# CNR-STIIMA-IRAS/rosdyn

Hardware: NVIDIA B200
Metric: 6-DOF regressor+torque samples/sec (fp64) (higher is better)
Workload: dtype f64

## Files before the change

### rosdyn_b200/csrc/gram_common.cuh

```cuda
#pragma once
#ifndef __CUDACC_RTC__
#include <cuda_runtime.h>
#endif

#include "chain_dev.h"
#include "spatial.cuh"

namespace rdb
{

constexpr int GF_KSPLIT = 4;
constexpr int GF_MMA_WARPS = 2 * GF_KSPLIT;
constexpr int GF_GENS = GF_KSPLIT;
constexpr int GF_THREADS = 32 * (GF_MMA_WARPS + GF_GENS);
constexpr int GF_MAX_SLOTS = 4;
constexpr int GF_BAR_REDUCE = 1;

__device__ __forceinline__ void bar_sync(int id, int count) { asm volatile("bar.sync %0, %1;" ::"r"(id), "r"(count) : "memory"); }
__device__ __forceinline__ void dmma884f(double& d0, double& d1, double a, double b)
{
  asm volatile("mma.sync.aligned.m8n8k4.row.col.f64.f64.f64.f64 {%0,%1}, {%2}, {%3}, {%0,%1};\n" : "+d"(d0), "+d"(d1) : "d"(a), "d"(b));
}
__device__ __forceinline__ uint32_t smem_u32(const void* p) { return (uint32_t)__cvta_generic_to_shared(p); }

template <int V>
struct ic
{
  static constexpr int value = V;
};
template <int B, int E, class F>
__device__ __forceinline__ void static_for(F&& f)
{
  if constexpr (B < E)
  {
    f(ic<B>{});
    static_for<B + 1, E>(f);
  }
}

constexpr int GX_COLS = 8;
template <int NJ, int Z = 0>
struct GramGeom
{
  static constexpr int P = 10 * NJ;
  static constexpr int TC = Z == 2 ? 0 : 1;
  __host__ __device__ static constexpr int inblk(int p)
  {
    constexpr int zord[10] = {9, 1, 2, 8, 3, 4, 5, 6, 7, 0};
    return Z == 2 ? zord[p] : (Z == 1 ? (p == 0 ? 9 : p - 1) : p);
  }
  __host__ __device__ static constexpr int param_at(int q)
  {
    constexpr int zinv[10] = {9, 1, 2, 4, 5, 6, 7, 8, 3, 0};
    return Z == 2 ? zinv[q] : (Z == 1 ? (q == 9 ? 0 : q + 1) : q);
  }
  __host__ __device__ static constexpr int pos(int l, int p) { return TC + 10 * (NJ - 1 - l) + inblk(p); }
  __host__ __device__ static constexpr bool stored(int j, int l, int p)
  {
    if (j != l || Z == 0) return true;
    if (Z == 1) return p != 0;
    return l == 0 ? (p == 1 || p == 2 || p == 9) : (p != 0 && p != 3);
  }
  __host__ __device__ static constexpr int rowlen(int j)
  {
    return Z == 2 ? TC + 10 * (NJ - 1 - j) + (j == 0 ? 3 : 8) : 1 + 10 * (NJ - j) - Z;
  }
  static constexpr int NPOS = rowlen(0);
  __host__ __device__ static constexpr int col_of(int q) { return q < TC ? P : 10 * (NJ - 1 - (q - TC) / 10) + param_at((q - TC) % 10); }
  __host__ __device__ static constexpr bool has_pos(int c) { return c / 10 > 0 || stored(0, 0, c % 10); }
  static constexpr int T = (NPOS + 7) / 8;
  static constexpr int NT = T * (T + 1) / 2;
  static constexpr int NF = T + 1 - TC;
  static constexpr int PARTIAL = NT * 64 + (TC ? 0 : 8 * T + 1);
  static constexpr int KPW = 8 / GF_KSPLIT;
  static constexpr int NSTEPS = NJ * KPW;
  __host__ __device__ static constexpr int rowbase(int j)
  {
    int o = 0;
    for (int i = 0; i < j; i++) o += rowlen(i) * 32;
    return o;
  }
  __host__ __device__ static constexpr int taubase(int j) { return TC ? rowbase(j) : rowbase(NJ) + 32 * j; }
  static constexpr int SLOT_DOUBLES = rowbase(NJ) + (TC ? 0 : 32 * NJ);
  __host__ __device__ static constexpr int tile(int I, int J) { return I * T - I * (I - 1) / 2 + (J - I); }
  __host__ __device__ static constexpr bool owns(int I, int par) { return (I & 1) == par; }
  __host__ __device__ static constexpr int ntiles(int par)
  {
    int n = 0;
    for (int I = 0; I < T; I++)
      if (owns(I, par)) n += T - I;
    return n > 0 ? n : 1;
  }
  __host__ __device__ static constexpr int local(int I, int J, int par)
  {
    int n = 0;
    for (int K = 0; K < I; K++)
      if (owns(K, par)) n += T - K;
    return n + (J - I);
  }
  __host__ __device__ static constexpr int bown(int I, int par)
  {
    int n = 0;
    for (int K = 0; K < I; K++)
      if (owns(K, par)) n++;
    return n;
  }
  __host__ __device__ static constexpr int nbacc(int par) { return TC || (par != 0 && bown(T, par) == 0) ? 1 : bown(T, par) + (par == 0 ? 1 : 0); }
  __host__ __device__ static constexpr int tj(int j) { return (rowlen(j) + 7) / 8; }
  __host__ __device__ static constexpr int xtile(int j, int I)
  {
    int n = 0;
    for (int k = 0; k < j; k++) n += tj(k) + 1;
    return n + I;
  }
  __host__ __device__ static constexpr int nxt()
  {
    int n = 0;
    for (int k = 0; k < NJ; k++) n += tj(k) + 1;
    return n;
  }
  static constexpr int NXT = nxt();
  __host__ __device__ static constexpr bool xowns(int j, int I, int par) { return ((I == tj(j) ? j : I) & 1) == par; }
  __host__ __device__ static constexpr int xlocal(int j, int I, int par)
  {
    int n = 0;
    for (int k = 0; k <= j; k++)
      for (int K = 0; K <= tj(k); K++)
      {
        if (k == j && K == I) return n;
        if (xowns(k, K, par)) n++;
      }
    return n;
  }
  __host__ __device__ static constexpr int nxtiles(int par)
  {
    int n = 0;
    for (int k = 0; k < NJ; k++)
      for (int K = 0; K <= tj(k); K++)
        if (xowns(k, K, par)) n++;
    return n;
  }
};

enum : int
{
  GXK_SAT = 1,
  GXK_OMEGA = 2,
  GXK_SGN = 3,
  GXK_SQ = 4,
  GXK_Q = 5,
  GXK_ONE = 6
};
struct GramComps
{
  int32_t ncols[8];
  int32_t kind[8][GX_COLS];
  double thr[8][GX_COLS], vmax[8][GX_COLS];
  double ithr[8][GX_COLS];
};

struct RtModel
{
  static constexpr bool RUNTIME = true;
};
enum : int
{
  MK_A = 0,
  MK_T = 1,
  MK_PI = 2,
  MK_G = 3
};
struct Zr
{
};
template <int S>
struct Un
{
};
template <class T>
struct tv_unit
{
  static constexpr int s = 0;
};
template <int S>
struct tv_unit<Un<S>>
{
  static constexpr int s = S;
};
template <class T>
struct tv_zero
{
  static constexpr bool v = false;
};
template <>
struct tv_zero<Zr>
{
  static constexpr bool v = true;
};

template <class M, int F, int L, int K, int NJ>
__device__ __forceinline__ auto kc(const ChainDev<NJ>& C)
{
  if constexpr (M::RUNTIME)
  {
    if constexpr (F == MK_A) return C.joint[L].A[K];
    else if constexpr (F == MK_T) return C.joint[L].t[K];
    else if constexpr (F == MK_PI) return C.link[L].pi[K];
    else return C.g[K];
  }
  else
  {
    constexpr double v = M::val(F, L, K);
    if constexpr (v == 0.0) return Zr{};
    else if constexpr (v == 1.0) return Un<1>{};
    else if constexpr (v == -1.0) return Un<-1>{};
    else return v;
  }
}

template <class A>
__device__ __forceinline__ double tv_d(A a)
{
  if constexpr (tv_zero<A>::v) return 0.0;
  else if constexpr (tv_unit<A>::s != 0) return (double)tv_unit<A>::s;
  else return a;
}
template <class A>
__device__ __forceinline__ auto tneg(A a)
{
  if constexpr (tv_zero<A>::v) return Zr{};
  else if constexpr (tv_unit<A>::s != 0) return Un<-tv_unit<A>::s>{};
  else return -a;
}
template <class A, class B>
__device__ __forceinline__ auto tmul(A a, B b)
{
  constexpr int ua = tv_unit<A>::s, ub = tv_unit<B>::s;
  if constexpr (tv_zero<A>::v || tv_zero<B>::v) return Zr{};
  else if constexpr (ua != 0 && ub != 0) return Un<ua * ub>{};
  else if constexpr (ua != 0) return ua > 0 ? b : -b;
  else if constexpr (ub != 0) return ub > 0 ? a : -a;
  else return __dmul_rn(a, b);
}
template <class A, class B>
__device__ __forceinline__ auto tadd(A a, B b)
{
  if constexpr (tv_zero<A>::v) return b;
  else if constexpr (tv_zero<B>::v) return a;
  else return __dadd_rn(tv_d(a), tv_d(b));
}
template <class A, class B, class C>
__device__ __forceinline__ auto tfma(A a, B b, C c)
{
  using P = decltype(tmul(a, b));
  if constexpr (tv_zero<P>::v) return c;
  else if constexpr (tv_zero<C>::v) return tmul(a, b);
  else if constexpr (tv_unit<A>::s != 0 || tv_unit<B>::s != 0) return tadd(tmul(a, b), c);
  else return __fma_rn(a, b, tv_d(c));
}

// ... 75 lines not shown
    if (G::stored(J, L, p))
      o[G::pos(L, p) * 32 + (lane ^ (4 * (G::pos(L, p) & 3)))] = e[p];
}
template <class M, int NJ, int Z, int L, int J, class U, class S>
__device__ __forceinline__ void gram_project(const ChainDev<NJ>& C, double (&tau)[NJ], double* __restrict__ slot, int lane, const U& u, const S& s,
                                             const V3& fm, const V3& w, const V3& al)
{
  const auto h = tcross_add(tcross_add(tcross(u, al), w, tcross(w, u)), fm, s);
  const auto rho = tcross(s, w);
  gram_emit<M, NJ, Z, L, J, false>(
      C, tau, slot, lane, tdot(u, fm), h.x, h.y, h.z, tfma(s.x, al.x, tmul(rho.x, w.x)),
      tfma(s.x, al.y, tfma(s.y, al.x, tfma(rho.x, w.y, tmul(rho.y, w.x)))), tfma(s.x, al.z, tfma(s.z, al.x, tfma(rho.x, w.z, tmul(rho.z, w.x)))),
      tfma(s.y, al.y, tmul(rho.y, w.y)), tfma(s.y, al.z, tfma(s.z, al.y, tfma(rho.y, w.z, tmul(rho.z, w.y)))), tfma(s.z, al.z, tmul(rho.z, w.z)));
}

template <int NJ, class M, int Z>
__device__ __forceinline__ void gram_walk_rev(const ChainDev<NJ>& C, const GenIn<NJ>& x, double* __restrict__ slot, int lane, double (&tau)[NJ])
{
  static_assert(REV_AXIS[0] == 0.0 && REV_AXIS[1] == 0.0 && REV_AXIS[2] == 1.0, "the REV walk below is written for the axis s = e_z");
  V3 U[NJ], S[NJ];
  V3 v = v3(0, 0, 0), w = v3(0, 0, 0), a = v3(0, 0, 0), al = v3(0, 0, 0), g;
  static_for<0, NJ>([&](auto lc) {
    constexpr int l = decltype(lc)::value;
    const double dql = x.dq[l], ddql = x.ddq[l];
    const double sl = x.sv[l], cl = x.cv[l];
    const auto t = mk3(kc<M, MK_T, l, 0>(C), kc<M, MK_T, l, 1>(C), kc<M, MK_T, l, 2>(C));
    auto row = [&](auto kc_) {
      constexpr int k = decltype(kc_)::value;
      const auto a0 = kc<M, MK_A, l, 3 * k>(C);
      const auto a1 = kc<M, MK_A, l, 3 * k + 1>(C);
      return mk3(tfma(sl, a1, tmul(cl, a0)), tfma(-sl, a0, tmul(cl, a1)), kc<M, MK_A, l, 3 * k + 2>(C));
    };
    const auto R = mk3(row(ic<0>{}), row(ic<1>{}), row(ic<2>{}));
    v = tod3(trotT(R, tcross_add(v, w, t)));
    w = tod3(trotT(R, w));
    a = tod3(trotT(R, tcross_add(a, al, t)));
    al = tod3(trotT(R, al));
    if constexpr (l == 0) g = tod3(trotT(R, mk3(kc<M, MK_G, 0, 0>(C), kc<M, MK_G, 0, 1>(C), kc<M, MK_G, 0, 2>(C))));
    else g = tod3(trotT(R, g));
    w.z += dql;
    a.x = fma(v.y, dql, a.x);
    a.y = fma(-v.x, dql, a.y);
    al.x = fma(w.y, dql, al.x);
    al.y = fma(-w.x, dql, al.y);
    al.z += ddql;
    static_for<0, (l > 0 ? l - 1 : 0)>([&](auto jc) {
      constexpr int j = decltype(jc)::value;
      U[j] = tod3(trotT(R, tcross_add(U[j], S[j], t)));
      S[j] = tod3(trotT(R, S[j]));
    });
    const auto S1 = R.z;
    const auto U1 = mk3(tfma(t.x, R.y.x, tneg(tmul(t.y, R.x.x))), tfma(t.x, R.y.y, tneg(tmul(t.y, R.x.y))), tfma(t.x, R.y.z, tneg(tmul(t.y, R.x.z))));
    if constexpr (l > 0)
    {
      S[l - 1] = tod3(S1);
      U[l - 1] = tod3(U1);
    }
    const V3 fm = cross_add(a - g, w, v);
    static_for<0, l + 1>([&](auto jc) {
      constexpr int j = decltype(jc)::value;
      if constexpr (j == l)
      {
        const double e7 = w.x * w.y;
        gram_emit<M, NJ, Z, l, j, true>(C, tau, slot, lane, Zr{}, fm.y, -fm.x, Zr{}, -e7, fma(w.x, w.x, -(w.y * w.y)), fma(-w.y, w.z, al.x),
                                        e7, fma(w.x, w.z, al.y), al.z);
      }
      else if constexpr (j == l - 1) gram_project<M, NJ, Z, l, j>(C, tau, slot, lane, U1, S1, fm, w, al);
      else gram_project<M, NJ, Z, l, j>(C, tau, slot, lane, U[j], S[j], fm, w, al);
    });
  });
}

template <int NJ, int Z>
__device__ __forceinline__ void gram_walk_gen(const ChainDev<NJ>& C, const GenIn<NJ>& x, double* __restrict__ slot, int lane, double (&tau)[NJ])
{
  using G = GramGeom<NJ, Z>;
  V3 U[NJ], S[NJ];
  V3 v = v3(0, 0, 0), w = v3(0, 0, 0), a = v3(0, 0, 0), al = v3(0, 0, 0);
  V3 g = v3(C.g);
#pragma unroll
  for (int l = 0; l < NJ; l++)
  {
    const JointDev& J = C.joint[l];
    const double dql = x.dq[l], ddql = x.ddq[l];
    double R[9];
    const V3 t = J.type != RDB_JOINT_PRISMATIC ? v3(J.t) : axpy(v3(J.t), v3(J.axp), x.q[l]);
    if (J.type == RDB_JOINT_REVOLUTE)
    {
      const double c1 = 1.0 - x.cv[l];
#pragma unroll
      for (int k = 0; k < 9; k++) R[k] = fma(c1, J.C[k], fma(x.sv[l], J.B[k], J.A[k]));
    }
    else
    {
#pragma unroll
      for (int k = 0; k < 9; k++) R[k] = J.A[k];
    }
    v = rotT(R, cross_add(v, w, t));
    w = rotT(R, w);
    a = rotT(R, cross_add(a, al, t));
    al = rotT(R, al);
    g = rotT(R, g);
    const V3 axj = v3(J.ax);
    const V3 su = J.type == RDB_JOINT_PRISMATIC ? axj : v3(0, 0, 0);
    const V3 ss = J.type == RDB_JOINT_REVOLUTE ? axj : v3(0, 0, 0);
    v = axpy(v, su, dql);
    w = axpy(w, ss, dql);
    const V3 xl = cross_add(cross(w, su), v, ss);
    const V3 xa = cross(w, ss);
    a = axpy(axpy(a, xl, dql), su, ddql);
    al = axpy(axpy(al, xa, dql), ss, ddql);
    U[l] = su;
    S[l] = ss;
#pragma unroll
    for (int j = 0; j < l; j++)
    {
      U[j] = rotT(R, cross_add(U[j], S[j], t));
      S[j] = rotT(R, S[j]);
    }
    tau[l] = 0.0;
    const double* Pl = C.link[l].pi;
    const V3 fm = cross_add(a - g, w, v);
#pragma unroll
    for (int j = 0; j <= l; j++)
    {
      const V3 u = U[j], s = S[j];
      const V3 h = cross_add(cross_add(cross(u, al), w, cross(w, u)), fm, s);
      const V3 rho = cross(s, w);
      double e[10];
      e[0] = dot(u, fm);
      e[1] = h.x;
      e[2] = h.y;
      e[3] = h.z;
      e[4] = fma(s.x, al.x, rho.x * w.x);
      e[5] = fma(s.x, al.y, fma(s.y, al.x, fma(rho.x, w.y, rho.y * w.x)));
      e[6] = fma(s.x, al.z, fma(s.z, al.x, fma(rho.x, w.z, rho.z * w.x)));
      e[7] = fma(s.y, al.y, rho.y * w.y);
      e[8] = fma(s.y, al.z, fma(s.z, al.y, fma(rho.y, w.z, rho.z * w.y)));
      e[9] = fma(s.z, al.z, rho.z * w.z);
      double t0 = tau[j], t1 = e[1] * Pl[1];
#pragma unroll
      for (int p = 0; p < 10; p += 2) t0 = fma(e[p], Pl[p], t0);
#pragma unroll
      for (int p = 3; p < 10; p += 2) t1 = fma(e[p], Pl[p], t1);
      tau[j] = t0 + t1;
      double* o = slot + G::rowbase(j);
#pragma unroll
      for (int p = 0; p < 10; p++) o[G::pos(l, p) * 32 + (lane ^ (4 * (G::pos(l, p) & 3)))] = e[p];
    }
  }
}

template <int NJ, bool REV, int Z, class M>
__device__ __forceinline__ void gram_generate(const ChainDev<NJ>& C, const GenIn<NJ>& x, const SamplesDev& in, const double* __restrict__ tau_meas,
                                              double* __restrict__ slot, int64_t i, int lane)
{
  static_assert(!Z || REV, "the zero mass column of a link on its own joint exists for revolute joints only");
  static_assert(REV || M::RUNTIME, "compile-time models are built for the REV walk");
  using G = GramGeom<NJ, Z>;
  double tau[NJ];
  if constexpr (REV) gram_walk_rev<NJ, M, Z>(C, x, slot, lane, tau);
  else gram_walk_gen<NJ, Z>(C, x, slot, lane, tau);
#pragma unroll
  for (int j = 0; j < NJ; j++)
  {
    const double tv = tau_meas ? __ldcs(tau_meas + (int64_t)C.joint[j].in * in.ld + i) : tau[j];
    slot[G::taubase(j) + lane] = tv;
  }
}

template <int NJ, int Z>
__device__ __noinline__ void gram_zero_lane(double* __restrict__ slot, int lane)
{
  using G = GramGeom<NJ, Z>;
  for (int j = 0; j < NJ; j++)
  {
    for (int c = 0; c < G::rowlen(j); c++) slot[G::rowbase(j) + c * 32 + (lane ^ (4 * (c & 3)))] = 0.0;
    if (!G::TC) slot[G::taubase(j) + lane] = 0.0;
  }
}

}
```

### rosdyn_b200/csrc/gram_fused.cu

```cuda
#include <cuda_runtime.h>

#include <algorithm>
#include <cstdio>
#include <cstdlib>
#include <type_traits>
#include <vector>

#include "gram_fused.cuh"
#include "launch.h"

namespace rdb
{

template <int NJ, int Z>
__global__ void gram_fused_reduce_kernel(const double* __restrict__ partial, int nparts, int pstride, double* __restrict__ gram,
                                         double* __restrict__ rhs, double* __restrict__ tau_sq, int accumulate)
{
  using G = GramGeom<NJ, Z>;
  constexpr int P = G::P;
  const int e = blockIdx.x * blockDim.x + threadIdx.x;
  if (!accumulate && e < P * (P + 1))
  {
    const int c = e / (P + 1), r = e % (P + 1);
    if (!G::has_pos(c))
    {
      if (r == P) rhs[c] = 0.0;
      else
      {
        gram[(size_t)c * P + r] = 0.0;
        gram[(size_t)r * P + c] = 0.0;
      }
    }
  }
  if (e >= G::PARTIAL) return;
  double s = 0.0;
  for (int p = 0; p < nparts; p++) s += partial[(size_t)p * pstride + e];
  if (e >= G::NT * 64)
  {
    const int q = e - G::NT * 64;
    if (q == 8 * G::T)
    {
      if (tau_sq) *tau_sq = accumulate ? *tau_sq + s : s;
    }
    else if (q < G::NPOS)
    {
      const int a = G::col_of(q);
      rhs[a] = accumulate ? rhs[a] + s : s;
    }
    return;
  }
  int k = e >> 6, I = 0;
  while (k >= G::T - I)
  {
    k -= G::T - I;
    I++;
  }
  const int J = I + k;
  const int rp = 8 * I + ((e >> 3) & 7), cp = 8 * J + (e & 7);
  if (rp >= G::NPOS || cp >= G::NPOS) return;
  if (I == J && rp > cp) return;
  const int row = G::col_of(rp), col = G::col_of(cp);
  if (row < P && col < P)
  {
    const double v = accumulate ? gram[(size_t)col * P + row] + s : s;
    gram[(size_t)col * P + row] = v;
    if (row != col) gram[(size_t)row * P + col] = v;
  }
  else if (row < P || col < P)
  {
    const int a = row < P ? row : col;
    rhs[a] = accumulate ? rhs[a] + s : s;
  }
  else if (tau_sq)
    *tau_sq = accumulate ? *tau_sq + s : s;
}
template <int NJ, int Z>
static void launch_fused_reduce(const double* partial, int nparts, int pstride, double* gram, double* rhs, double* tau_sq, int accumulate,
                                cudaStream_t st)
{
  using G = GramGeom<NJ, Z>;
  const int n = std::max(G::PARTIAL, G::P * (G::P + 1));
  gram_fused_reduce_kernel<NJ, Z><<<(n + 255) / 256, 256, 0, st>>>(partial, nparts, pstride, gram, rhs, tau_sq, accumulate);
  count_launch();
}

__global__ void gram_fold_expand_kernel(const double* __restrict__ T, const int32_t* __restrict__ kof, const double* __restrict__ Gr,
                                        const double* __restrict__ br, const double* __restrict__ tsr, int nj, int Pr, double* __restrict__ gram,
                                        double* __restrict__ rhs, double* __restrict__ tau_sq, int accumulate)
{
  const int P = 10 * nj;
  const int e = blockIdx.x * blockDim.x + threadIdx.x;
  if (e >= P * (P + 1)) return;
  const int a = e / (P + 1), b = e % (P + 1);
  if (e == P && tau_sq) *tau_sq = accumulate ? *tau_sq + *tsr : *tsr;
  if (b < a) return;
  const int la = a / 10, pa = a % 10, ka = kof[la];
  double s = 0.0;
  if (b == P)
  {
    if (ka >= 0)
      for (int c = 0; c < 10; c++) s = fma(T[(size_t)la * 100 + c * 10 + pa], br[10 * ka + c], s);
    rhs[a] = accumulate ? rhs[a] + s : s;
    return;
  }
  const int lb = b / 10, pb = b % 10, kb = kof[lb];
  if (ka >= 0 && kb >= 0)
    for (int c = 0; c < 10; c++)
    {
      double r = 0.0;
      for (int d = 0; d < 10; d++) r = fma(Gr[(size_t)(10 * kb + d) * Pr + 10 * ka + c], T[(size_t)lb * 100 + d * 10 + pb], r);
      s = fma(T[(size_t)la * 100 + c * 10 + pa], r, s);
    }
  const double v = accumulate ? gram[(size_t)b * P + a] + s : s;
  gram[(size_t)b * P + a] = v;
  if (a != b) gram[(size_t)a * P + b] = v;
}

static int gram_dev_switch()
{
#ifdef RDB_DEV_SWITCHES
  static const int dbg = [] { const char* e = getenv("RDB_GRAM_DEBUG"); return e ? atoi(e) : 0; }();
  return dbg;
#else
  return 0;
#endif
}

cudaError_t launch_fold_expand(ChainHost& ch, double* gram, double* rhs, double* tau_sq, int accumulate, cudaStream_t st)
{
  const int nj = ch.host.nj, Pr = 10 * ch.gram.fold.nj, P = 10 * nj;
  double* Tm = ch.gram.fold_dev;
  double* Gr = Tm + (size_t)nj * 100;
  double* br = Gr + (size_t)Pr * Pr;
  double* tsr = br + Pr;
  const int32_t* kof = reinterpret_cast<const int32_t*>(Gr + (size_t)(Pr + 1) * (Pr + 1));
  gram_fold_expand_kernel<<<(P * (P + 1) + 127) / 128, 128, 0, st>>>(Tm, kof, Gr, br, tsr, nj, Pr, gram, rhs, tau_sq, accumulate);
  count_launch();
  return cudaGetLastError();
}

template <int NJ>
static ChainDev<NJ> narrow_g(const ChainDev<RDB_MAX_JOINTS>& h)
{
  ChainDev<NJ> c;
  c.nj = h.nj;
  c.n_in = h.n_in;
  for (int k = 0; k < 3; k++) c.g[k] = h.g[k];
  for (int j = 0; j < NJ; j++)
  {
    c.joint[j] = h.joint[j];
    c.link[j] = h.link[j];
  }
  return c;
}

static cudaError_t grow(double*& p, size_t& have, size_t need)
{
  if (have >= need) return cudaSuccess;
  if (p) cudaFree(p);
  p = nullptr;
  have = 0;
  cudaError_t e = cudaMalloc(&p, need);
  if (e == cudaSuccess) have = need;
  return e;
}

template <int NJ, int Z, int XC>
constexpr int gf_slots()
{
  return std::min<int>(GF_MAX_SLOTS,
                       (int)((227 * 1024 - 1024) / (sizeof(double) * (GramGeom<NJ, Z>::SLOT_DOUBLES + gram_ext_side_doubles<NJ, XC>()))));
}

template <int NJ, bool REV, int XC>
static cudaError_t launch_fused_kernel(ChainHost& ch, const GramComps& gc, const SamplesDev& in, const double* tau_meas, double* partials,
                                       int* grid, cudaStream_t st)
{
  constexpr int Z = REV ? (XC ? 1 : 2) : 0;
  constexpr int SLOTS = gf_slots<NJ, Z, XC>();
  static_assert(SLOTS >= 2, "the fused kernel needs two slots");
  const void* kfn = reinterpret_cast<const void*>(gram_fused_kernel<NJ, SLOTS, REV, XC>);
  if (REV)
  {
    char args[64];
    snprintf(args, sizeof args, "gram_fused_kernel<%d, %d, true, %d", NJ, SLOTS, XC);
    if (const void* jk = gram_jit_kernel(ch, args)) kfn = jk;
  }
  else
  {
    ch.gram.kernel_specialised = 0;
    ch.gram.kernel_why = "precompiled kernel: not every folded joint is revolute about e_z (generic generator)";
  }
  const size_t smem = sizeof(double) * (size_t)gram_smem_doubles<NJ, Z, SLOTS, XC>();
  cudaError_t e = cudaFuncSetAttribute(kfn, cudaFuncAttributeMaxDynamicSharedMemorySize, (int)smem);
  if (e != cudaSuccess) return e;
  const int64_t ngroups = (in.n + 31) / 32;
  constexpr int B = gram_group_block<SLOTS, XC>();
  *grid = (int)std::min<int64_t>(ch.sm_count, (ngroups + B - 1) / B);
  ChainDev<NJ> C = narrow_g<NJ>(ch.gram.fold);
  GramComps comps = gc;
  SamplesDev ins = in;
  const double* tm = tau_meas;
  double* part = partials;
  int dbg = gram_dev_switch();
  void* args[] = {&C, &comps, &ins, &tm, &part, &dbg};
  e = cudaLaunchKernel(kfn, dim3(*grid), dim3(GF_THREADS), args, smem, st);
  if (e != cudaSuccess) return e;
  count_launch();
  return cudaSuccess;
}

template <int NJ, bool REV>
static cudaError_t launch_fused_nj(ChainHost& ch, const SamplesDev& in, const double* tau_meas, double* gram, double* rhs, double* tau_sq,
                                   int accumulate, cudaStream_t st)
{
  constexpr int Z = REV ? 2 : 0;
  using G = GramGeom<NJ, Z>;
  cudaError_t e = grow(ch.gram.fused_partials, ch.gram.fused_bytes, sizeof(double) * (size_t)ch.sm_count * G::PARTIAL);
  if (e != cudaSuccess) return e;
  int grid = 0;
  e = launch_fused_kernel<NJ, REV, 0>(ch, GramComps{}, in, tau_meas, ch.gram.fused_partials, &grid, st);
  if (e != cudaSuccess) return e;
  if (ch.gram.fold_identity)
  {
    launch_fused_reduce<NJ, Z>(ch.gram.fused_partials, grid, G::PARTIAL, gram, rhs, tau_sq, accumulate, st);
    return cudaGetLastError();
  }
  const int nj = ch.host.nj, Pr = G::P;
  double* Tm = ch.gram.fold_dev;
  double* Gr = Tm + (size_t)nj * 100;
  double* br = Gr + (size_t)Pr * Pr;
  double* tsr = br + Pr;
  launch_fused_reduce<NJ, Z>(ch.gram.fused_partials, grid, G::PARTIAL, Gr, br, tsr, 0, st);
  return launch_fold_expand(ch, gram, rhs, tau_sq, accumulate, st);
}

cudaError_t launch_gram_fused(ChainHost& ch, const SamplesDev& in, const double* tau_meas, double* gram, double* rhs, double* tau_sq,
                              int accumulate, cudaStream_t st)
{
  if (in.n <= 0 || ch.gram.fold_version != ch.model_version) return cudaErrorNotSupported;
  const bool rev = fold_rev_canonical(ch.gram.fold);
  switch (ch.gram.fold.nj)
  {
#define X(N)                                                                                  \
  case N:                                                                                     \
    return rev ? launch_fused_nj<N, true>(ch, in, tau_meas, gram, rhs, tau_sq, accumulate, st) \
               : launch_fused_nj<N, false>(ch, in, tau_meas, gram, rhs, tau_sq, accumulate, st);
    X(1) X(2) X(3) X(4) X(5) X(6) X(7)
#undef X
  }
  return cudaErrorNotSupported;
}

__global__ void gram_cross_reduce_kernel(const double* __restrict__ partial, int nparts, int n, int pstride, double* __restrict__ sum)
{
  const int e = blockIdx.x * blockDim.x + threadIdx.x;
  if (e >= n) return;
  double s = 0.0;
  for (int p = 0; p < nparts; p++) s += partial[(size_t)p * pstride + e];
  sum[e] = s;
}

__global__ void gram_ext_scatter_kernel(const double* __restrict__ G, const double* __restrict__ b, const double* __restrict__ ts, int P, int Pt,
                                        double* __restrict__ gram, double* __restrict__ rhs, double* __restrict__ tau_sq, int accumulate)
{
  const int e = blockIdx.x * blockDim.x + threadIdx.x;
  if (e >= P * (P + 1)) return;
  const int a = e / (P + 1), c = e % (P + 1);
  if (e == P && tau_sq) *tau_sq = accumulate ? *tau_sq + *ts : *ts;
  if (c == P)
  {
    rhs[a] = accumulate ? rhs[a] + b[a] : b[a];
    return;
  }
  const double v = G[(size_t)c * P + a];
  gram[(size_t)c * Pt + a] = accumulate ? gram[(size_t)c * Pt + a] + v : v;
}

template <int NJ, int Z>
__global__ void gram_cross_finish_kernel(const double* __restrict__ X, const double* __restrict__ Tm, const int32_t* __restrict__ kof,
                                         const int32_t* __restrict__ xj, const int32_t* __restrict__ xs, int nj, int Pc, double* __restrict__ gram,
                                         double* __restrict__ rhs, int accumulate)
{
  using G = GramGeom<NJ, Z>;
  static_assert(G::TC == 1, "tau is the tile column at position 0");
  const int P = 10 * nj, Pt = P + Pc;
  const int e = blockIdx.x * blockDim.x + threadIdx.x;
  if (e >= (P + 1 + Pc) * Pc) return;
  const int a = e / Pc, cc = e % Pc;
  const int j = xj[cc], g = xs[cc];
  const int tb = G::xtile(j, 0);
  auto xval = [&](int col) -> double {
    const int pos = col == G::P ? 0 : G::pos(col / 10, col % 10);
    return pos >= G::rowlen(j) ? 0.0 : X[(size_t)(tb + (pos >> 3)) * 64 + (pos & 7) * 8 + g];
  };
  if (a < P)
  {
    double s = 0.0;
    if (kof)
    {
      const int la = a / 10, pa = a % 10, ka = kof[la];
      if (ka >= 0)
        for (int c = 0; c < 10; c++) s = fma(Tm[(size_t)la * 100 + c * 10 + pa], xval(10 * ka + c), s);
    }
    else
      s = xval(a);
    double* o = gram + (size_t)(P + cc) * Pt + a;
    const double v = accumulate ? *o + s : s;
    *o = v;
    gram[(size_t)a * Pt + P + cc] = v;
  }
  else if (a == P)
  {
    const double s = xval(G::P);
    rhs[P + cc] = accumulate ? rhs[P + cc] + s : s;
  }
  else
  {
    const int c2 = a - P - 1;
    const double s = (xj[c2] == j) ? X[(size_t)(tb + G::tj(j)) * 64 + xs[c2] * 8 + g] : 0.0;
    double* o = gram + (size_t)(P + cc) * Pt + P + c2;
    *o = accumulate ? *o + s : s;
  }
}
// ... 121 lines not shown
```

### rosdyn_b200/csrc/gram_fused.cuh

```cuda
#pragma once
#include "gram_common.cuh"

namespace rdb
{

constexpr int GF_POLL_NS = 32;
struct GramBars
{
  uint64_t full[GF_MAX_SLOTS], empty[GF_MAX_SLOTS];
  uint32_t filled[GF_MAX_SLOTS];
  uint32_t drained[GF_MAX_SLOTS];
};
__device__ __forceinline__ void mbarrier_init(uint64_t* b, int count)
{
  asm volatile("mbarrier.init.shared::cta.b64 [%0], %1;" ::"r"(smem_u32(b)), "r"(count) : "memory");
}
__device__ __forceinline__ void mbarrier_arrive(uint64_t* b)
{
  asm volatile("{\n .reg .b64 st;\n mbarrier.arrive.shared::cta.b64 st, [%0];\n}" ::"r"(smem_u32(b)) : "memory");
}
__device__ __forceinline__ void mbarrier_wait(uint64_t* b, uint32_t parity)
{
  asm volatile(
      "{\n .reg .pred p;\n"
      "W: mbarrier.try_wait.parity.shared::cta.b64 p, [%0], %1;\n"
      " @p bra D;\n bra W;\n"
      "D:\n}" ::"r"(smem_u32(b)),
      "r"(parity)
      : "memory");
}
__device__ __forceinline__ uint32_t ld_acquire_u32(const uint32_t* p)
{
  uint32_t v;
  asm volatile("ld.acquire.cta.shared.u32 %0, [%1];" : "=r"(v) : "r"(smem_u32(p)) : "memory");
  return v;
}
__device__ __forceinline__ void st_release_u32(uint32_t* p, uint32_t v)
{
  asm volatile("st.release.cta.shared.u32 [%0], %1;" ::"r"(smem_u32(p)), "r"(v) : "memory");
}
__device__ __forceinline__ void red_release_inc(uint32_t* p)
{
  asm volatile("red.release.cta.shared.add.u32 [%0], 1;" ::"r"(smem_u32(p)) : "memory");
}
__device__ __forceinline__ void wait_counter_ge(const uint32_t* p, uint32_t v)
{
  while (ld_acquire_u32(p) < v) __nanosleep(GF_POLL_NS);
}

template <int SLOTS, int XC>
__host__ __device__ constexpr int gram_group_block()
{
  return XC == 0 && SLOTS == GF_GENS ? SLOTS : 1;
}
template <int B>
__device__ __forceinline__ int64_t gram_group(int64_t k)
{
  return ((k / B) * gridDim.x + blockIdx.x) * B + k % B;
}
template <int B>
__device__ __forceinline__ int64_t gram_cta_groups(int64_t ngroups)
{
  if constexpr (B == 1) return ngroups > blockIdx.x ? (ngroups - blockIdx.x + gridDim.x - 1) / gridDim.x : 0;
  const int64_t nb = (ngroups + B - 1) / B;
  if (nb <= blockIdx.x) return 0;
  const int64_t q = (nb - 1 - blockIdx.x) / gridDim.x;
  return q * B + min((int64_t)B, ngroups - (q * gridDim.x + blockIdx.x) * B);
}

template <int NJ, int XC>
__host__ __device__ constexpr int gram_ext_side_doubles()
{
  return NJ * XC * 32;
}
template <int NJ, int XC>
__device__ __forceinline__ void gram_component_park(const GenIn<NJ>& x, double* __restrict__ side, int lane)
{
  static_assert(XC >= 2, "q and Dq of a joint are staged in its first two columns");
#pragma unroll
  for (int j = 0; j < NJ; j++)
  {
    side[(j * XC) * 32 + lane] = x.dq[j];
    side[(j * XC + 1) * 32 + lane] = x.q[j];
  }
}
template <int NJ, int XC>
__device__ __forceinline__ void gram_component_side(const GramComps& comps, double* __restrict__ side, int lane)
{
#pragma unroll 1
  for (int j = 0; j < NJ; j++)
  {
    double* o = side + (j * XC) * 32 + lane;
    const double dq = o[0], q = o[32];
    const int nc = comps.ncols[j];
#pragma unroll(XC <= 4 ? XC : 1)
    for (int c = 0; c < XC; c++)
    {
      double val = 0.0;
      if (c < nc)
      {
        const int kd = comps.kind[j][c];
        const double th = comps.thr[j][c], vm = comps.vmax[j][c];
        const double omega = fmin(fmax(dq, -vm), vm);
        if (kd == GXK_OMEGA) val = omega;
        else if (kd == GXK_Q) val = q;
        else if (kd == GXK_ONE) val = 1.0;
        else
        {
          const double r = omega * comps.ithr[j][c];
          if (kd == GXK_SAT) val = fmin(fmax(r, -1.0), 1.0);
          else
          {
            const double sg = omega == 0.0 ? 0.0 : (omega > th ? 1.0 : (omega < -th ? -1.0 : r));
            val = kd == GXK_SGN ? sg : omega * omega * sg;
          }
        }
      }
      o[c * 32] = val;
    }
  }
}

template <int NJ, int Z, int XC>
__host__ __device__ constexpr int gram_partial_doubles()
{
  return GramGeom<NJ, Z>::PARTIAL + (XC ? GramGeom<NJ, Z>::NXT * 64 : 0);
}
template <int NJ, int Z, int SLOTS, int XC>
__host__ __device__ constexpr int gram_side_offset()
{
  return GramGeom<NJ, Z>::SLOT_DOUBLES * SLOTS > gram_partial_doubles<NJ, Z, XC>() ? GramGeom<NJ, Z>::SLOT_DOUBLES * SLOTS
                                                                                   : gram_partial_doubles<NJ, Z, XC>();
}
template <int NJ, int Z, int SLOTS, int XC>
__host__ __device__ constexpr int gram_smem_doubles()
{
  return gram_side_offset<NJ, Z, SLOTS, XC>() + SLOTS * gram_ext_side_doubles<NJ, XC>();
}

template <int NJ, int SLOTS, bool REV, int Z, int XC, class M>
__device__ __forceinline__ void gram_gen_role(const ChainDev<NJ>& C, const GramComps& comps, const SamplesDev& in, const double* __restrict__ tau_meas,
                                              double* smem, double* side0, GramBars* bars, int w, int lane, int dbg)
{
  using G = GramGeom<NJ, Z>;
  constexpr int B = gram_group_block<SLOTS, XC>();
  const int64_t nk = gram_cta_groups<B>((in.n + 31) / 32);
  for (int64_t k = w; k < nk; k += GF_GENS)
  {
    const int s = (int)(k % SLOTS);
    const uint32_t u = (uint32_t)(k / SLOTS);
    const int64_t i = gram_group<B>(k) * 32 + lane;
    GenIn<NJ> cur;
    gen_load<NJ>(C, in, min(i, in.n - 1), cur);
    trig_all<NJ>(cur.q, cur.sv, cur.cv);
    if constexpr (B == SLOTS) mbarrier_wait(&bars->empty[s], (u & 1) ^ 1);
    else wait_counter_ge(&bars->drained[s], GF_MMA_WARPS * u);
    double* slot = smem + (size_t)s * G::SLOT_DOUBLES;
    double* side = side0 + (size_t)s * gram_ext_side_doubles<NJ, XC>();
    if (XC > 0 || !(dbg & 1))
    {
      if constexpr (XC > 0) gram_component_park<NJ, XC>(cur, side, lane);
      gram_generate<NJ, REV, Z, M>(C, cur, in, tau_meas, slot, min(i, in.n - 1), lane);
      if constexpr (XC > 0) gram_component_side<NJ, XC>(comps, side, lane);
      if (i >= in.n)
      {
        gram_zero_lane<NJ, Z>(slot, lane);
        for (int c = 0; c < NJ * XC; c++) side[c * 32 + lane] = 0.0;
      }
    }
    __syncwarp();
    if (lane == 0)
    {
      if constexpr (B == SLOTS) mbarrier_arrive(&bars->full[s]);
      else st_release_u32(&bars->filled[s], u + 1);
    }
  }
}

template <int NJ, int J, int Z>
__device__ __forceinline__ void gram_load_frags(const double* __restrict__ slot, int kk, int lane, double (&b)[GramGeom<NJ, Z>::NF])
{
  using G = GramGeom<NJ, Z>;
  constexpr int T = G::T, L = G::rowlen(J), TJ = G::tj(J);
  const int g = lane >> 2, t = lane & 3;
  const double* rowp = slot + G::rowbase(J) + ((4 * kk + t) ^ (4 * (g & 3)));
#pragma unroll
  for (int I = 0; I < T; I++)
  {
    if (I >= TJ) continue;
    const int col = 8 * I + g;
    if (8 * I + 7 < L || col < L) b[I] = rowp[col * 32];
    else b[I] = 0.0;
  }
  if constexpr (!G::TC) b[T] = slot[G::taubase(J) + 4 * kk + t];
}
template <int J, int XC>
__device__ __forceinline__ double gram_load_xside(const double* __restrict__ side, int kk, int lane)
{
  const int g = lane >> 2, t = lane & 3;
  return g < XC ? side[(J * XC + g) * 32 + 4 * kk + t] : 0.0;
}
template <int NJ, int PAR, int J, int Z>
__device__ __forceinline__ void gram_mma_step(const double (&b)[GramGeom<NJ, Z>::NF], double (&acc)[GramGeom<NJ, Z>::ntiles(PAR)][2])
{
  using G = GramGeom<NJ, Z>;
  constexpr int T = G::T, TJ = G::tj(J);
#pragma unroll
  for (int I = 0; I < T; I++)
  {
    if (I >= TJ || !G::owns(I, PAR)) continue;
#pragma unroll
    for (int K = I; K < T; K++)
      if (K < TJ) dmma884f(acc[G::local(I, K, PAR)][0], acc[G::local(I, K, PAR)][1], b[I], b[K]);
  }
}
template <int NJ, int PAR, int J, int Z>
__device__ __forceinline__ void gram_tau_step(const double (&b)[GramGeom<NJ, Z>::NF], double (&bacc)[GramGeom<NJ, Z>::nbacc(PAR)])
{
  using G = GramGeom<NJ, Z>;
  static_for<0, G::tj(J)>([&](auto Ic) {
    constexpr int I = decltype(Ic)::value;
    if constexpr (G::owns(I, PAR)) bacc[G::bown(I, PAR)] = fma(b[I], b[G::T], bacc[G::bown(I, PAR)]);
  });
  if constexpr (PAR == 0) bacc[G::nbacc(PAR) - 1] = fma(b[G::T], b[G::T], bacc[G::nbacc(PAR) - 1]);
}
template <int NJ, int PAR, int J, int Z, int NX>
__device__ __forceinline__ void gram_cross_step(const double (&b)[GramGeom<NJ, Z>::NF], double bx, double (&xacc)[NX][2])
{
  using G = GramGeom<NJ, Z>;
  static_for<0, G::tj(J) + 1>([&](auto Ic) {
    constexpr int I = decltype(Ic)::value;
    if constexpr (G::xowns(J, I, PAR))
    {
      constexpr int k = G::xlocal(J, I, PAR);
      if constexpr (I < G::tj(J)) dmma884f(xacc[k][0], xacc[k][1], b[I], bx);
      else dmma884f(xacc[k][0], xacc[k][1], bx, bx);
    }
  });
}
template <int NJ, int PAR, int STEP, int Z, int XC, int NX>
__device__ __forceinline__ void gram_consume_steps(const double* __restrict__ slot, const double* __restrict__ side, int ks, int lane,
                                                   const double (&bcur)[GramGeom<NJ, Z>::NF], double bxcur,
                                                   double (&acc)[GramGeom<NJ, Z>::ntiles(PAR)][2], double (&bacc)[GramGeom<NJ, Z>::nbacc(PAR)],
                                                   double (&xacc)[NX][2])
{
  using G = GramGeom<NJ, Z>;
  constexpr int J = STEP / G::KPW;
  double bnext[G::NF], bxnext = 0.0;
  if constexpr (STEP + 1 < G::NSTEPS)
  {
    constexpr int JN = (STEP + 1) / G::KPW;
    const int kn = ks * G::KPW + (STEP + 1) % G::KPW;
    gram_load_frags<NJ, JN, Z>(slot, kn, lane, bnext);
    if constexpr (XC > 0) bxnext = gram_load_xside<JN, XC>(side, kn, lane);
  }
  gram_mma_step<NJ, PAR, J, Z>(bcur, acc);
  if constexpr (!G::TC) gram_tau_step<NJ, PAR, J, Z>(bcur, bacc);
  if constexpr (XC > 0) gram_cross_step<NJ, PAR, J, Z>(bcur, bxcur, xacc);
  if constexpr (STEP + 1 < G::NSTEPS) gram_consume_steps<NJ, PAR, STEP + 1, Z, XC>(slot, side, ks, lane, bnext, bxnext, acc, bacc, xacc);
}

template <int NJ, int PAR, int Z>
__device__ __forceinline__ void gram_mma_reduce(double (&acc)[GramGeom<NJ, Z>::ntiles(PAR)][2], double* smem, int ks, int lane)
{
  using G = GramGeom<NJ, Z>;
  bar_sync(GF_BAR_REDUCE, 32 * GF_MMA_WARPS);
  const int g = lane >> 2, t = lane & 3;
  for (int w = 0; w < GF_KSPLIT; w++)
  {
    if (ks == w)
    {
#pragma unroll
      for (int I = 0; I < G::T; I++)
      {
        if (!G::owns(I, PAR)) continue;
#pragma unroll
        for (int J = I; J < G::T; J++)
        {
          double* o = smem + G::tile(I, J) * 64 + g * 8 + 2 * t;
          const int k = G::local(I, J, PAR);
          if (w == 0)
          {
            o[0] = acc[k][0];
            o[1] = acc[k][1];
          }
          else
          {
            o[0] += acc[k][0];
            o[1] += acc[k][1];
          }
        }
      }
    }
    bar_sync(GF_BAR_REDUCE, 32 * GF_MMA_WARPS);
  }
}
template <int NJ, int PAR, int Z>
__device__ __forceinline__ void gram_tau_reduce(double (&bacc)[GramGeom<NJ, Z>::nbacc(PAR)], double* smem, int ks, int lane)
{
  using G = GramGeom<NJ, Z>;
  constexpr int NB = G::nbacc(PAR);
#pragma unroll
  for (int k = 0; k < NB; k++)
  {
    bacc[k] += __shfl_xor_sync(0xffffffffu, bacc[k], 1);
    bacc[k] += __shfl_xor_sync(0xffffffffu, bacc[k], 2);
  }
  const int g = lane >> 2, t = lane & 3;
  double* ob = smem + G::NT * 64;
  for (int w = 0; w < GF_KSPLIT; w++)
  {
    if (ks == w && t == 0)
    {
#pragma unroll
      for (int I = 0; I < G::T; I++)
      {
        if (!G::owns(I, PAR)) continue;
        double& o = ob[8 * I + g];
        o = w == 0 ? bacc[G::bown(I, PAR)] : o + bacc[G::bown(I, PAR)];
      }
      if (PAR == 0 && g == 0) ob[8 * G::T] = w == 0 ? bacc[NB - 1] : ob[8 * G::T] + bacc[NB - 1];
    }
    bar_sync(GF_BAR_REDUCE, 32 * GF_MMA_WARPS);
  }
}
template <int NJ, int PAR, int Z, int NX>
__device__ __forceinline__ void gram_cross_reduce_smem(double (&xacc)[NX][2], double* smem, int ks, int lane)
{
  using G = GramGeom<NJ, Z>;
  bar_sync(GF_BAR_REDUCE, 32 * GF_MMA_WARPS);
  const int g = lane >> 2, t = lane & 3;
  for (int w = 0; w < GF_KSPLIT; w++)
  {
    if (ks == w)
    {
      static_for<0, NJ>([&](auto jc) {
        constexpr int j = decltype(jc)::value;
        static_for<0, G::tj(j) + 1>([&](auto Ic) {
          constexpr int I = decltype(Ic)::value;
          if constexpr (G::xowns(j, I, PAR))
          {
            double* o = smem + G::xtile(j, I) * 64 + g * 8 + 2 * t;
            constexpr int k = G::xlocal(j, I, PAR);
            if (w == 0)
            {
              o[0] = xacc[k][0];
              o[1] = xacc[k][1];
            }
            else
            {
              o[0] += xacc[k][0];
              o[1] += xacc[k][1];
            }
          }
        });
      });
    }
    bar_sync(GF_BAR_REDUCE, 32 * GF_MMA_WARPS);
  }
}

template <int NJ, int SLOTS, int PAR, int Z, int XC>
__device__ __forceinline__ void gram_mma_role(const SamplesDev& in, double* smem, const double* side0, GramBars* bars, int ks, int lane, int dbg)
{
  using G = GramGeom<NJ, Z>;
  constexpr int B = gram_group_block<SLOTS, XC>();
  constexpr int NTP = G::ntiles(PAR), NB = G::nbacc(PAR), NX = XC ? G::nxtiles(PAR) : 1;
  double acc[NTP][2], bacc[NB], xacc[NX][2];
#pragma unroll
  for (int k = 0; k < NTP; k++) acc[k][0] = acc[k][1] = 0.0;
#pragma unroll
  for (int k = 0; k < NB; k++) bacc[k] = 0.0;
#pragma unroll
  for (int k = 0; k < NX; k++) xacc[k][0] = xacc[k][1] = 0.0;
  const int64_t nk = gram_cta_groups<B>((in.n + 31) / 32);
#pragma unroll 1
  for (int64_t k = 0; k < nk; k++)
  {
    const int s = (int)(k % SLOTS);
    const uint32_t u = (uint32_t)(k / SLOTS);
    const double* slot = smem + (size_t)s * G::SLOT_DOUBLES;
    const double* side = side0 + (size_t)s * gram_ext_side_doubles<NJ, XC>();
    if constexpr (B == SLOTS) mbarrier_wait(&bars->full[s], u & 1);
    else wait_counter_ge(&bars->filled[s], u + 1);
    if (XC > 0 || !(dbg & 2))
    {
      double b0[G::NF], bx0 = 0.0;
      gram_load_frags<NJ, 0, Z>(slot, ks * G::KPW, lane, b0);
      if constexpr (XC > 0) bx0 = gram_load_xside<0, XC>(side, ks * G::KPW, lane);
      gram_consume_steps<NJ, PAR, 0, Z, XC>(slot, side, ks, lane, b0, bx0, acc, bacc, xacc);
    }
    __syncwarp();
    if (lane == 0)
    {
      if constexpr (B == SLOTS) mbarrier_arrive(&bars->empty[s]);
      else red_release_inc(&bars->drained[s]);
    }
  }
  gram_mma_reduce<NJ, PAR, Z>(acc, smem, ks, lane);
  if constexpr (!G::TC) gram_tau_reduce<NJ, PAR, Z>(bacc, smem, ks, lane);
  if constexpr (XC > 0) gram_cross_reduce_smem<NJ, PAR, Z>(xacc, smem + G::NT * 64, ks, lane);
}

template <int NJ, int SLOTS, bool REV, int XC, class M = RtModel>
__global__ void __launch_bounds__(GF_THREADS, 1)
    gram_fused_kernel(const __grid_constant__ ChainDev<NJ> C, const __grid_constant__ GramComps comps, const SamplesDev in,
                      const double* __restrict__ tau_meas, double* __restrict__ partial, const int dbg)
{
  constexpr int Z = REV ? (XC ? 1 : 2) : 0;
  using G = GramGeom<NJ, Z>;
  constexpr int NOUT = gram_partial_doubles<NJ, Z, XC>();
  extern __shared__ __align__(16) double smem[];
  __shared__ GramBars bars;
  double* const side0 = smem + gram_side_offset<NJ, Z, SLOTS, XC>();
  const int warp = threadIdx.x >> 5, lane = threadIdx.x & 31;
  if constexpr (gram_group_block<SLOTS, XC>() == SLOTS)
  {
    if (threadIdx.x == 0)
    {
      for (int s = 0; s < SLOTS; s++)
      {
        mbarrier_init(&bars.full[s], 1);
        mbarrier_init(&bars.empty[s], GF_MMA_WARPS);
      }
      asm volatile("fence.mbarrier_init.release.cluster;" ::: "memory");
    }
  }
  else if (threadIdx.x < SLOTS)
  {
    bars.filled[threadIdx.x] = 0;
    bars.drained[threadIdx.x] = 0;
  }
  __syncthreads();
  if (warp >= GF_MMA_WARPS)
  {
    gram_gen_role<NJ, SLOTS, REV, Z, XC, M>(C, comps, in, tau_meas, smem, side0, &bars, warp - GF_MMA_WARPS, lane, dbg);
    return;
  }
  const int mma_id = warp, ks = mma_id % GF_KSPLIT;
  if (mma_id < GF_KSPLIT) gram_mma_role<NJ, SLOTS, 0, Z, XC>(in, smem, side0, &bars, ks, lane, dbg);
  else gram_mma_role<NJ, SLOTS, 1, Z, XC>(in, smem, side0, &bars, ks, lane, dbg);
  double* out = partial + (size_t)blockIdx.x * NOUT;
  for (int k = mma_id * 32 + lane; k < NOUT; k += 32 * GF_MMA_WARPS) out[k] = smem[k];
}

}
```

Before: 2.323 billion.

## Move torque projection accumulation from MMA warps to generator warps

The Gram-vs-torque products (A^T tau and tau^T tau) are no longer folded into the MMA warps' fragment loop. Generator warps now compute them on FP64 CUDA cores right after filling each slot and accumulate per-warp partials in a new shared-memory region. A named barrier joins generators and MMA warps before the final reduce, and the extra generator drain is counted in the slot-release protocol. This lightens MMA-warp register pressure and per-step FMA work, but adds generator work, an extra slot-release dependency, and shared memory that may reduce the slot count.

```diff
diff --git a/rosdyn_b200/csrc/gram_common.cuh b/rosdyn_b200/csrc/gram_common.cuh
--- a/rosdyn_b200/csrc/gram_common.cuh
+++ b/rosdyn_b200/csrc/gram_common.cuh
@@ -15,8 +15,10 @@
 constexpr int GF_THREADS = 32 * (GF_MMA_WARPS + GF_GENS);
 constexpr int GF_MAX_SLOTS = 4;
 constexpr int GF_BAR_REDUCE = 1;
+constexpr int GF_BAR_GENS = 2;
 
 __device__ __forceinline__ void bar_sync(int id, int count) { asm volatile("bar.sync %0, %1;" ::"r"(id), "r"(count) : "memory"); }
+__device__ __forceinline__ void bar_arrive(int id, int count) { asm volatile("bar.arrive %0, %1;" ::"r"(id), "r"(count) : "memory"); }
 __device__ __forceinline__ void dmma884f(double& d0, double& d1, double a, double b)
 {
   asm volatile("mma.sync.aligned.m8n8k4.row.col.f64.f64.f64.f64 {%0,%1}, {%2}, {%3}, {%0,%1};\n" : "+d"(d0), "+d"(d1) : "d"(a), "d"(b));
@@ -70,7 +72,7 @@
   __host__ __device__ static constexpr bool has_pos(int c) { return c / 10 > 0 || stored(0, 0, c % 10); }
   static constexpr int T = (NPOS + 7) / 8;
   static constexpr int NT = T * (T + 1) / 2;
-  static constexpr int NF = T + 1 - TC;
+  static constexpr int NF = T;
   static constexpr int PARTIAL = NT * 64 + (TC ? 0 : 8 * T + 1);
   static constexpr int KPW = 8 / GF_KSPLIT;
   static constexpr int NSTEPS = NJ * KPW;
@@ -98,14 +100,6 @@
       if (owns(K, par)) n += T - K;
     return n + (J - I);
   }
-  __host__ __device__ static constexpr int bown(int I, int par)
-  {
-    int n = 0;
-    for (int K = 0; K < I; K++)
-      if (owns(K, par)) n++;
-    return n;
-  }
-  __host__ __device__ static constexpr int nbacc(int par) { return TC || (par != 0 && bown(T, par) == 0) ? 1 : bown(T, par) + (par == 0 ? 1 : 0); }
   __host__ __device__ static constexpr int tj(int j) { return (rowlen(j) + 7) / 8; }
   __host__ __device__ static constexpr int xtile(int j, int I)
   {
@@ -487,13 +481,13 @@
 }
 
 template <int NJ, bool REV, int Z, class M>
-__device__ __forceinline__ void gram_generate(const ChainDev<NJ>& C, const GenIn<NJ>& x, const SamplesDev& in, const double* __restrict__ tau_meas,
-                                              double* __restrict__ slot, int64_t i, int lane)
+__device__ __forceinline__ double gram_generate(const ChainDev<NJ>& C, const GenIn<NJ>& x, const SamplesDev& in, const double* __restrict__ tau_meas,
+                                                double* __restrict__ slot, int64_t i, int lane)
 {
   static_assert(!Z || REV, "the zero mass column of a link on its own joint exists for revolute joints only");
   static_assert(REV || M::RUNTIME, "compile-time models are built for the REV walk");
   using G = GramGeom<NJ, Z>;
-  double tau[NJ];
+  double tau[NJ], tsq = 0.0;
   if constexpr (REV) gram_walk_rev<NJ, M, Z>(C, x, slot, lane, tau);
   else gram_walk_gen<NJ, Z>(C, x, slot, lane, tau);
 #pragma unroll
@@ -501,7 +495,9 @@
   {
     const double tv = tau_meas ? __ldcs(tau_meas + (int64_t)C.joint[j].in * in.ld + i) : tau[j];
     slot[G::taubase(j) + lane] = tv;
-  }
+    tsq = fma(tv, tv, tsq);
+  }
+  return tsq;
 }
 
 template <int NJ, int Z>
diff --git a/rosdyn_b200/csrc/gram_fused.cu b/rosdyn_b200/csrc/gram_fused.cu
--- a/rosdyn_b200/csrc/gram_fused.cu
+++ b/rosdyn_b200/csrc/gram_fused.cu
@@ -168,8 +168,8 @@
 template <int NJ, int Z, int XC>
 constexpr int gf_slots()
 {
-  return std::min<int>(GF_MAX_SLOTS,
-                       (int)((227 * 1024 - 1024) / (sizeof(double) * (GramGeom<NJ, Z>::SLOT_DOUBLES + gram_ext_side_doubles<NJ, XC>()))));
+  return std::min<int>(GF_MAX_SLOTS, (int)((227 * 1024 - 1024 - sizeof(double) * gram_tau_acc_doubles<NJ, Z>()) /
+                                           (sizeof(double) * (GramGeom<NJ, Z>::SLOT_DOUBLES + gram_ext_side_doubles<NJ, XC>()))));
 }
 
 template <int NJ, bool REV, int XC>
diff --git a/rosdyn_b200/csrc/gram_fused.cuh b/rosdyn_b200/csrc/gram_fused.cuh
--- a/rosdyn_b200/csrc/gram_fused.cuh
+++ b/rosdyn_b200/csrc/gram_fused.cuh
@@ -11,6 +11,11 @@
   uint32_t filled[GF_MAX_SLOTS];
   uint32_t drained[GF_MAX_SLOTS];
 };
+template <int TC>
+__host__ __device__ constexpr int gram_drainers()
+{
+  return GF_MMA_WARPS + (TC ? 0 : 1);
+}
 __device__ __forceinline__ void mbarrier_init(uint64_t* b, int count)
 {
   asm volatile("mbarrier.init.shared::cta.b64 [%0], %1;" ::"r"(smem_u32(b)), "r"(count) : "memory");
@@ -132,18 +137,74 @@
   return GramGeom<NJ, Z>::SLOT_DOUBLES * SLOTS > gram_partial_doubles<NJ, Z, XC>() ? GramGeom<NJ, Z>::SLOT_DOUBLES * SLOTS
                                                                                    : gram_partial_doubles<NJ, Z, XC>();
 }
+template <int NJ, int Z>
+__host__ __device__ constexpr int gram_tau_acc_doubles()
+{
+  return GramGeom<NJ, Z>::TC ? 0 : GF_GENS * (GramGeom<NJ, Z>::T + 1) * 32;
+}
 template <int NJ, int Z, int SLOTS, int XC>
 __host__ __device__ constexpr int gram_smem_doubles()
 {
-  return gram_side_offset<NJ, Z, SLOTS, XC>() + SLOTS * gram_ext_side_doubles<NJ, XC>();
+  return gram_side_offset<NJ, Z, SLOTS, XC>() + SLOTS * gram_ext_side_doubles<NJ, XC>() + gram_tau_acc_doubles<NJ, Z>();
+}
+
+template <int NJ, int Z>
+__device__ __forceinline__ void gram_tau_pass(const double* __restrict__ slot, double tsq, double* __restrict__ tacc, int lane)
+{
+  using G = GramGeom<NJ, Z>;
+  constexpr int T = G::T;
+  const int g = lane >> 2, t = lane & 3;
+  double b0[T], b1[T];
+#pragma unroll
+  for (int I = 0; I < T; I++) b0[I] = b1[I] = 0.0;
+#pragma unroll
+  for (int m = 0; m < 8; m += 2)
+  {
+    const int c0 = 4 * (m ^ (g & 3)) + t, c1 = 4 * ((m + 1) ^ (g & 3)) + t;
+    static_for<0, NJ>([&](auto jc) {
+      constexpr int J = decltype(jc)::value, L = G::rowlen(J);
+      const double* rowp = slot + G::rowbase(J);
+      const double t0 = slot[G::taubase(J) + 4 * m + t], t1 = slot[G::taubase(J) + 4 * m + 4 + t];
+#pragma unroll
+      for (int I = 0; I < G::tj(J); I++)
+      {
+        const int col = 8 * I + g;
+        if (8 * I + 7 < L || col < L)
+        {
+          b0[I] = fma(rowp[col * 32 + c0], t0, b0[I]);
+          b1[I] = fma(rowp[col * 32 + c1], t1, b1[I]);
+        }
+      }
+    });
+  }
+#pragma unroll
+  for (int I = 0; I < T; I++) tacc[I * 32 + lane] += b0[I] + b1[I];
+  tacc[T * 32 + lane] += tsq;
+}
+template <int NJ, int Z>
+__device__ __forceinline__ double gram_tau_sum(const double* __restrict__ tacc0, int q)
+{
+  using G = GramGeom<NJ, Z>;
+  constexpr int W = (G::T + 1) * 32;
+  const int I = q >> 3, n = q < 8 * G::T ? 4 : 32;
+  const double* a = tacc0 + (q < 8 * G::T ? I * 32 + 4 * (q & 7) : G::T * 32);
+  double s = 0.0;
+  for (int w = 0; w < GF_GENS; w++)
+    for (int l = 0; l < n; l++) s += a[w * W + l];
+  return s;
 }
 
 template <int NJ, int SLOTS, bool REV, int Z, int XC, class M>
 __device__ __forceinline__ void gram_gen_role(const ChainDev<NJ>& C, const GramComps& comps, const SamplesDev& in, const double* __restrict__ tau_meas,
-                                              double* smem, double* side0, GramBars* bars, int w, int lane, int dbg)
+                                              double* smem, double* side0, double* tacc, GramBars* bars, int w, int lane, int dbg)
 {
   using G = GramGeom<NJ, Z>;
   constexpr int B = gram_group_block<SLOTS, XC>();
+  if constexpr (!G::TC)
+  {
+#pragma unroll 1
+    for (int I = 0; I <= G::T; I++) tacc[I * 32 + lane] = 0.0;
+  }
   const int64_t nk = gram_cta_groups<B>((in.n + 31) / 32);
   for (int64_t k = w; k < nk; k += GF_GENS)
   {
@@ -154,18 +215,20 @@
     gen_load<NJ>(C, in, min(i, in.n - 1), cur);
     trig_all<NJ>(cur.q, cur.sv, cur.cv);
     if constexpr (B == SLOTS) mbarrier_wait(&bars->empty[s], (u & 1) ^ 1);
-    else wait_counter_ge(&bars->drained[s], GF_MMA_WARPS * u);
+    else wait_counter_ge(&bars->drained[s], gram_drainers<G::TC>() * u);
     double* slot = smem + (size_t)s * G::SLOT_DOUBLES;
     double* side = side0 + (size_t)s * gram_ext_side_doubles<NJ, XC>();
+    double tsq = 0.0;
     if (XC > 0 || !(dbg & 1))
     {
       if constexpr (XC > 0) gram_component_park<NJ, XC>(cur, side, lane);
-      gram_generate<NJ, REV, Z, M>(C, cur, in, tau_meas, slot, min(i, in.n - 1), lane);
+      tsq = gram_generate<NJ, REV, Z, M>(C, cur, in, tau_meas, slot, min(i, in.n - 1), lane);
       if constexpr (XC > 0) gram_component_side<NJ, XC>(comps, side, lane);
       if (i >= in.n)
       {
         gram_zero_lane<NJ, Z>(slot, lane);
         for (int c = 0; c < NJ * XC; c++) side[c * 32 + lane] = 0.0;
+        tsq = 0.0;
       }
     }
     __syncwarp();
@@ -173,6 +236,13 @@
     {
       if constexpr (B == SLOTS) mbarrier_arrive(&bars->full[s]);
       else st_release_u32(&bars->filled[s], u + 1);
+    }
+    if constexpr (!G::TC)
+    {
+      if (!(dbg & 1)) gram_tau_pass<NJ, Z>(slot, tsq, tacc, lane);
+      __syncwarp();
+      if constexpr (B != SLOTS)
+        if (lane == 0) red_release_inc(&bars->drained[s]);
     }
   }
 }
@@ -192,7 +262,6 @@
     if (8 * I + 7 < L || col < L) b[I] = rowp[col * 32];
     else b[I] = 0.0;
   }
-  if constexpr (!G::TC) b[T] = slot[G::taubase(J) + 4 * kk + t];
 }
 template <int J, int XC>
 __device__ __forceinline__ double gram_load_xside(const double* __restrict__ side, int kk, int lane)
@@ -213,16 +282,6 @@
     for (int K = I; K < T; K++)
       if (K < TJ) dmma884f(acc[G::local(I, K, PAR)][0], acc[G::local(I, K, PAR)][1], b[I], b[K]);
   }
-}
-template <int NJ, int PAR, int J, int Z>
-__device__ __forceinline__ void gram_tau_step(const double (&b)[GramGeom<NJ, Z>::NF], double (&bacc)[GramGeom<NJ, Z>::nbacc(PAR)])
-{
-  using G = GramGeom<NJ, Z>;
-  static_for<0, G::tj(J)>([&](auto Ic) {
-    constexpr int I = decltype(Ic)::value;
-    if constexpr (G::owns(I, PAR)) bacc[G::bown(I, PAR)] = fma(b[I], b[G::T], bacc[G::bown(I, PAR)]);
-  });
-  if constexpr (PAR == 0) bacc[G::nbacc(PAR) - 1] = fma(b[G::T], b[G::T], bacc[G::nbacc(PAR) - 1]);
 }
 template <int NJ, int PAR, int J, int Z, int NX>
 __device__ __forceinline__ void gram_cross_step(const double (&b)[GramGeom<NJ, Z>::NF], double bx, double (&xacc)[NX][2])
@@ -241,8 +300,7 @@
 template <int NJ, int PAR, int STEP, int Z, int XC, int NX>
 __device__ __forceinline__ void gram_consume_steps(const double* __restrict__ slot, const double* __restrict__ side, int ks, int lane,
                                                    const double (&bcur)[GramGeom<NJ, Z>::NF], double bxcur,
-                                                   double (&acc)[GramGeom<NJ, Z>::ntiles(PAR)][2], double (&bacc)[GramGeom<NJ, Z>::nbacc(PAR)],
-                                                   double (&xacc)[NX][2])
+                                                   double (&acc)[GramGeom<NJ, Z>::ntiles(PAR)][2], double (&xacc)[NX][2])
 {
   using G = GramGeom<NJ, Z>;
   constexpr int J = STEP / G::KPW;
@@ -255,9 +313,8 @@
     if constexpr (XC > 0) bxnext = gram_load_xside<JN, XC>(side, kn, lane);
   }
   gram_mma_step<NJ, PAR, J, Z>(bcur, acc);
-  if constexpr (!G::TC) gram_tau_step<NJ, PAR, J, Z>(bcur, bacc);
   if constexpr (XC > 0) gram_cross_step<NJ, PAR, J, Z>(bcur, bxcur, xacc);
-  if constexpr (STEP + 1 < G::NSTEPS) gram_consume_steps<NJ, PAR, STEP + 1, Z, XC>(slot, side, ks, lane, bnext, bxnext, acc, bacc, xacc);
+  if constexpr (STEP + 1 < G::NSTEPS) gram_consume_steps<NJ, PAR, STEP + 1, Z, XC>(slot, side, ks, lane, bnext, bxnext, acc, xacc);
 }
 
 template <int NJ, int PAR, int Z>
@@ -291,35 +348,6 @@
           }
         }
       }
-    }
-    bar_sync(GF_BAR_REDUCE, 32 * GF_MMA_WARPS);
-  }
-}
-template <int NJ, int PAR, int Z>
-__device__ __forceinline__ void gram_tau_reduce(double (&bacc)[GramGeom<NJ, Z>::nbacc(PAR)], double* smem, int ks, int lane)
-{
-  using G = GramGeom<NJ, Z>;
-  constexpr int NB = G::nbacc(PAR);
-#pragma unroll
-  for (int k = 0; k < NB; k++)
-  {
-    bacc[k] += __shfl_xor_sync(0xffffffffu, bacc[k], 1);
-    bacc[k] += __shfl_xor_sync(0xffffffffu, bacc[k], 2);
-  }
-  const int g = lane >> 2, t = lane & 3;
-  double* ob = smem + G::NT * 64;
-  for (int w = 0; w < GF_KSPLIT; w++)
-  {
-    if (ks == w && t == 0)
-    {
-#pragma unroll
-      for (int I = 0; I < G::T; I++)
-      {
-        if (!G::owns(I, PAR)) continue;
-        double& o = ob[8 * I + g];
-        o = w == 0 ? bacc[G::bown(I, PAR)] : o + bacc[G::bown(I, PAR)];
-      }
-      if (PAR == 0 && g == 0) ob[8 * G::T] = w == 0 ? bacc[NB - 1] : ob[8 * G::T] + bacc[NB - 1];
     }
     bar_sync(GF_BAR_REDUCE, 32 * GF_MMA_WARPS);
   }
@@ -365,12 +393,10 @@
 {
   using G = GramGeom<NJ, Z>;
   constexpr int B = gram_group_block<SLOTS, XC>();
-  constexpr int NTP = G::ntiles(PAR), NB = G::nbacc(PAR), NX = XC ? G::nxtiles(PAR) : 1;
-  double acc[NTP][2], bacc[NB], xacc[NX][2];
+  constexpr int NTP = G::ntiles(PAR), NX = XC ? G::nxtiles(PAR) : 1;
+  double acc[NTP][2], xacc[NX][2];
 #pragma unroll
   for (int k = 0; k < NTP; k++) acc[k][0] = acc[k][1] = 0.0;
-#pragma unroll
-  for (int k = 0; k < NB; k++) bacc[k] = 0.0;
 #pragma unroll
   for (int k = 0; k < NX; k++) xacc[k][0] = xacc[k][1] = 0.0;
   const int64_t nk = gram_cta_groups<B>((in.n + 31) / 32);
@@ -388,7 +414,7 @@
       double b0[G::NF], bx0 = 0.0;
       gram_load_frags<NJ, 0, Z>(slot, ks * G::KPW, lane, b0);
       if constexpr (XC > 0) bx0 = gram_load_xside<0, XC>(side, ks * G::KPW, lane);
-      gram_consume_steps<NJ, PAR, 0, Z, XC>(slot, side, ks, lane, b0, bx0, acc, bacc, xacc);
+      gram_consume_steps<NJ, PAR, 0, Z, XC>(slot, side, ks, lane, b0, bx0, acc, xacc);
     }
     __syncwarp();
     if (lane == 0)
@@ -397,8 +423,8 @@
       else red_release_inc(&bars->drained[s]);
     }
   }
+  if constexpr (!G::TC) bar_sync(GF_BAR_GENS, GF_THREADS);
   gram_mma_reduce<NJ, PAR, Z>(acc, smem, ks, lane);
-  if constexpr (!G::TC) gram_tau_reduce<NJ, PAR, Z>(bacc, smem, ks, lane);
   if constexpr (XC > 0) gram_cross_reduce_smem<NJ, PAR, Z>(xacc, smem + G::NT * 64, ks, lane);
 }
 
@@ -413,6 +439,7 @@
   extern __shared__ __align__(16) double smem[];
   __shared__ GramBars bars;
   double* const side0 = smem + gram_side_offset<NJ, Z, SLOTS, XC>();
+  double* const tacc0 = side0 + SLOTS * gram_ext_side_doubles<NJ, XC>();
   const int warp = threadIdx.x >> 5, lane = threadIdx.x & 31;
   if constexpr (gram_group_block<SLOTS, XC>() == SLOTS)
   {
@@ -434,14 +461,25 @@
   __syncthreads();
   if (warp >= GF_MMA_WARPS)
   {
-    gram_gen_role<NJ, SLOTS, REV, Z, XC, M>(C, comps, in, tau_meas, smem, side0, &bars, warp - GF_MMA_WARPS, lane, dbg);
+    gram_gen_role<NJ, SLOTS, REV, Z, XC, M>(C, comps, in, tau_meas, smem, side0, tacc0 + (warp - GF_MMA_WARPS) * (G::T + 1) * 32, &bars,
+                                            warp - GF_MMA_WARPS, lane, dbg);
+    if constexpr (!G::TC) bar_arrive(GF_BAR_GENS, GF_THREADS);
     return;
   }
   const int mma_id = warp, ks = mma_id % GF_KSPLIT;
   if (mma_id < GF_KSPLIT) gram_mma_role<NJ, SLOTS, 0, Z, XC>(in, smem, side0, &bars, ks, lane, dbg);
   else gram_mma_role<NJ, SLOTS, 1, Z, XC>(in, smem, side0, &bars, ks, lane, dbg);
   double* out = partial + (size_t)blockIdx.x * NOUT;
-  for (int k = mma_id * 32 + lane; k < NOUT; k += 32 * GF_MMA_WARPS) out[k] = smem[k];
-}
-
-}
+  for (int k = mma_id * 32 + lane; k < NOUT; k += 32 * GF_MMA_WARPS)
+  {
+    if constexpr (!G::TC)
+      if (k >= G::NT * 64)
+      {
+        out[k] = gram_tau_sum<NJ, Z>(tacc0, k - G::NT * 64);
+        continue;
+      }
+    out[k] = smem[k];
+  }
+}
+
+}
```

Result: slower. 1.838 billion (median of 6 runs) (-20.9%).
